# fdarmon/wild_deep_mvs

Measured on AMD Instinct MI355X. Metric: cost-volume voxels/sec (BxDxHxW), MVSNet hot path, higher is better.
Workload: dtype bf16

## Files before the change

### wild_deep_mvs_amd/csrc/conv3d_sweep.hip

```cpp
#include "conv_common.h"
#include <type_traits>

namespace pscv {

struct SweepArgs : ConvIO {
    int D, Hh, W;
    int epi;
    const uint16_t* in2;
    int in2_cs, in2_co;
    int nth, ntw, ndc, dc;
    unsigned mg_th, mg_tw, mg_dc;
};

PSCV_PROF_BUFFER(sweep)
constexpr int SW_BW = 18;
constexpr int SW_VB = 64;
constexpr int SW_NSLOT = 6;
template <int TH> struct SwGeom {
    static constexpr int BH = TH + 2;
    static constexpr int PV = ((BH * SW_BW + 7) / 8) * 8;
    static constexpr int PB = PV * SW_VB;
    static constexpr int LDS = SW_NSLOT * PB;
    static constexpr int CHUNKS = BH * SW_BW * 4;
    static constexpr int THREADS = 32 * TH;
    static constexpr int NLD = (CHUNKS + THREADS - 1) / THREADS;
};

__device__ __forceinline__ int sw_lds_off(int v, int chunk) {
    return v * SW_VB + ((chunk ^ (((v >> 2) & 1) << 1)) << 4);
}

template <typename H, int SW_TH>
__global__ __launch_bounds__(32 * SW_TH, 2) void conv3d_sweep8_kernel(const SweepArgs a) {
    extern __shared__ __attribute__((aligned(16))) unsigned char smem[];
    using G = SwGeom<SW_TH>;
    constexpr int SW_PB = G::PB, SW_CHUNKS = G::CHUNKS, NTHR = G::THREADS, NLD = G::NLD;
    constexpr int R = 2;

    int wg = xcd_remap(blockIdx.x, gridDim.x);
    const int dci = fast_divmod(wg, a.ndc, a.mg_dc);
    const int twi = fast_divmod(wg, a.ntw, a.mg_tw);
    const int thi = fast_divmod(wg, a.nth, a.mg_th);
    const int b = wg;
    const int h0 = thi * SW_TH, w0 = twi * 16;
    const int dbeg = dci * a.dc, dend = min(a.D, dbeg + a.dc);

    const int tid = threadIdx.x, lane = tid & 63, wave = tid >> 6;
    const int n = lane & 15, g = lane >> 4;
    PSCV_PROF_BEGIN

    uint4 wf[4][9];
    {
        const uint4* wp = reinterpret_cast<const uint4*>(a.wpk);
#pragma unroll
        for (int p = 0; p < 4; ++p)
#pragma unroll
            for (int t = 0; t < 9; ++t) wf[p][t] = wp[(p * 9 + t) * 64 + lane];
    }

    const int row0 = wave * R;
    int boff[R + 2][3];
#pragma unroll
    for (int rr = 0; rr < R + 2; ++rr)
#pragma unroll
        for (int kw = 0; kw < 3; ++kw) boff[rr][kw] = sw_lds_off((row0 + rr) * SW_BW + n + kw, g);

    unsigned goff[NLD];
    int loff[NLD];
    bool lval[NLD];
    const long plane_stride = (long)a.Hh * a.W * a.in_cs;
    const unsigned plane_bytes = (unsigned)(plane_stride * 2 - a.in_co * 2);
    const uint16_t* inb = a.in + (long)b * a.D * plane_stride + a.in_co;
#pragma unroll
    for (int i = 0; i < NLD; ++i) {
        const int id = tid + NTHR * i;
        const int v = id >> 2, c = id & 3;
        const int bh = v / SW_BW, bw = v - bh * SW_BW;
        const int gh = h0 - 1 + bh, gw = w0 - 1 + bw;
        lval[i] = id < SW_CHUNKS;
        const bool gval = lval[i] && (unsigned)gh < (unsigned)a.Hh && (unsigned)gw < (unsigned)a.W;
        goff[i] = gval ? ((unsigned)(gh * a.W + gw) * (unsigned)a.in_cs + (unsigned)(c * 8)) * 2u : 0x7ffffff0u;
        loff[i] = sw_lds_off(v, c);
    }
    const int plane_hi = min(a.D - 1, dend);
    auto fetch = [&](int plane, uint4 (&reg)[NLD]) {
        const bool pv = plane >= 0 && plane <= plane_hi;
        const __amdgpu_buffer_rsrc_t rs = __builtin_amdgcn_make_buffer_rsrc(
            const_cast<uint16_t*>(inb + (long)(pv ? plane : 0) * plane_stride), (short)0, pv ? (int)plane_bytes : 0, 0x00020000);
#pragma unroll
        for (int i = 0; i < NLD; ++i)
            reg[i] = __builtin_bit_cast(uint4, __builtin_amdgcn_raw_buffer_load_b128(rs, (int)goff[i], 0, 0));
    };
    auto stash = [&](int ring, const uint4 (&reg)[NLD]) {
        unsigned char* sp = smem + ring * SW_PB;
#pragma unroll
        for (int i = 0; i < NLD; ++i)
            if (lval[i]) *reinterpret_cast<uint4*>(sp + loff[i]) = reg[i];
    };

    const int c0 = (g & 1) * 4;
    float sc[4], bi[4], fl[4];
#pragma unroll
    for (int k = 0; k < 4; ++k) {
        sc[k] = a.scale ? a.scale[c0 + k] : 1.0f;
        bi[k] = a.bias ? a.bias[c0 + k] : 0.0f;
        fl[k] = a.floor ? a.floor[c0 + k] : 0.0f;
    }

    {
        uint4 ra[NLD], rb[NLD];
        fetch(dbeg - 1, ra); fetch(dbeg, rb);
        stash(0, ra); stash(1, rb);
        fetch(dbeg + 1, ra); fetch(dbeg + 2, rb);
        stash(2, ra); stash(3, rb);
    }
    __syncthreads();
    PSCV_STAMP(0)

    auto pair = [&](auto ringc, const int d) {
        constexpr int RING = decltype(ringc)::value;
        uint4 na[NLD], nb[NLD];
        fetch(d + 3, na);
        fetch(d + 4, nb);
        __builtin_amdgcn_sched_barrier(0);
        PSCV_STAMP(1)

        f32x4 acc[R];
#pragma unroll
        for (int r = 0; r < R; ++r) acc[r] = f32x4{0.f, 0.f, 0.f, 0.f};
#pragma unroll
        for (int p = 0; p < 4; ++p) {
            constexpr int SL = (RING + 4 * SW_NSLOT) % SW_NSLOT;
            const unsigned char* sp = smem + ((SL + p) % SW_NSLOT) * SW_PB;
#pragma unroll
            for (int kh = 0; kh < 3; ++kh)
#pragma unroll
                for (int kw = 0; kw < 3; ++kw)
#pragma unroll
                    for (int r = 0; r < R; ++r) {
                        const uint4 xf = *reinterpret_cast<const uint4*>(sp + boff[r + kh][kw]);
                        acc[r] = Mfma<H>::run(wf[p][kh * 3 + kw], xf, acc[r]);
                    }
        }

        PSCV_STAMP(2)
        const int od = d + (g >> 1);
#pragma unroll
        for (int r = 0; r < R; ++r) {
            const int oh = h0 + row0 + r, ow = w0 + n;
            if (od < dend && oh < a.Hh && ow < a.W) {
                const long vox = (((long)b * a.D + od) * a.Hh + oh) * a.W + ow;
                float y[4];
#pragma unroll
                for (int k = 0; k < 4; ++k) {
                    y[k] = fmaf(acc[r][k], sc[k], bi[k]);
                    if (a.epi & PSCV_EPI_RELU_PRE) y[k] = relu_floor(y[k], fl[k]);
                }
                if (a.skip) {
                    const uint2 sv = *reinterpret_cast<const uint2*>(a.skip + vox * a.skip_cs + a.skip_co + c0);
                    y[0] += Half16<H>::lo(sv.x); y[1] += Half16<H>::hi(sv.x);
                    y[2] += Half16<H>::lo(sv.y); y[3] += Half16<H>::hi(sv.y);
                }
                if (a.epi & PSCV_EPI_RELU_POST) {
#pragma unroll
                    for (int k = 0; k < 4; ++k) y[k] = relu_floor(y[k], 0.0f);
                }
                if (a.out_f32) {
                    *reinterpret_cast<float4*>(reinterpret_cast<float*>(a.out) + vox * a.out_cs + a.out_co + c0) =
                        make_float4(y[0], y[1], y[2], y[3]);
                } else {
                    *reinterpret_cast<uint2*>(reinterpret_cast<uint16_t*>(a.out) + vox * a.out_cs + a.out_co + c0) =
                        make_uint2(Half16<H>::pack(y[0], y[1]), Half16<H>::pack(y[2], y[3]));
                }
            }
        }

        PSCV_STAMP(3)
        stash((RING + 4) % SW_NSLOT, na);
        stash((RING + 5) % SW_NSLOT, nb);
        PSCV_STAMP(4)
        __syncthreads();
        PSCV_STAMP(5)
    };
    for (int d = dbeg; d < dend; d += 6) {
        pair(std::integral_constant<int, 0>{}, d);
        if (d + 2 < dend) pair(std::integral_constant<int, 2>{}, d + 2);
        if (d + 4 < dend) pair(std::integral_constant<int, 4>{}, d + 4);
    }
    PSCV_PROF_END(sweep, blockIdx.x)
}


constexpr int KM_NSLOT = 3;
constexpr int KM_PV = 192;
constexpr int KM_PB = KM_PV * SW_VB;
constexpr int KM_LDS = KM_NSLOT * KM_PB + 96;
constexpr int KM_CHUNKS = 10 * SW_BW * 4;
constexpr int KM_NLD = (KM_CHUNKS + 255) / 256;

#ifdef PSCV_ABLATE
#define KM_ABL(bit) (a.in2_cs & (bit))
#else
#define KM_ABL(bit) false
#endif
__device__ __forceinline__ int km_lds_off(int v, int chunk) { return v * SW_VB + ((chunk ^ ((v >> 2) & 3)) << 4); }

template <typename H, bool SKIP, int PD>
__global__ __launch_bounds__(256, 3) void conv3d_sweep8_kdm_kernel(const SweepArgs a) {
    extern __shared__ __attribute__((aligned(16))) unsigned char smem[];
    constexpr int NLD = KM_NLD;

    int wg = xcd_remap(blockIdx.x, gridDim.x);
    const int dci = fast_divmod(wg, a.ndc, a.mg_dc);
    const int twi = fast_divmod(wg, a.ntw, a.mg_tw);
    const int thi = fast_divmod(wg, a.nth, a.mg_th);
    const int b = wg;
    const int h0 = thi * 8, w0 = twi * 16;
    const int dbeg = dci * a.dc, dend = min(a.D, dbeg + a.dc);

    const int tid = threadIdx.x, lane = tid & 63, wave = tid >> 6;
    const int half = lane >> 5, nn = lane & 31;
    const int quad = nn >> 2;
    const int rr = ((0x69 >> quad) & 1) ? 0 : 1;
    const int px = (quad >> 1) * 4 + (nn & 3);
    const int row0 = wave * 2;

    uint4 wf[9][2];
    {
        const uint4* wp = reinterpret_cast<const uint4*>(a.wpk);
        const int kdb = nn >> 3, co = nn & 7;
#pragma unroll
        for (int t = 0; t < 9; ++t)
#pragma unroll
            for (int h = 0; h < 2; ++h)
                wf[t][h] = kdb < 3 ? wp[(kdb * 9 + t) * 64 + (2 * h + half) * 16 + co] : make_uint4(0u, 0u, 0u, 0u);
    }

    int boff[3][3];
#pragma unroll
    for (int kh = 0; kh < 3; ++kh)
#pragma unroll
        for (int kw = 0; kw < 3; ++kw) boff[kh][kw] = km_lds_off((row0 + rr + kh) * SW_BW + px + kw, half);

    unsigned goff[NLD];
    static_assert(NLD == 3 && KM_CHUNKS > 512 && KM_CHUNKS <= 768, "three chunks per thread, the third one partial");
    const int loff0 = km_lds_off(tid >> 2, tid & 3);
    const bool lval_last = tid + 512 < KM_CHUNKS;
    const long plane_stride = (long)a.Hh * a.W * a.in_cs;
    const unsigned plane_bytes = (unsigned)(plane_stride * 2 - a.in_co * 2);
    const uint16_t* inb = a.in + (long)b * a.D * plane_stride + a.in_co;
#pragma unroll
    for (int i = 0; i < NLD; ++i) {
        const int id = tid + 256 * i;
        const int v = id >> 2, c = id & 3;
        const int bh = v / SW_BW, bw = v - bh * SW_BW;
        const int gh = h0 - 1 + bh, gw = w0 - 1 + bw;
        const bool gval = id < KM_CHUNKS && (unsigned)gh < (unsigned)a.Hh && (unsigned)gw < (unsigned)a.W;
        goff[i] = gval ? ((unsigned)(gh * a.W + gw) * (unsigned)a.in_cs + (unsigned)(c * 8)) * 2u : 0x7ffffff0u;
    }
    const int plane_hi = min(a.D - 1, dend);
    auto fetch = [&](int plane, uint4 (&reg)[NLD]) {
        const bool pv = plane >= 0 && plane <= plane_hi;
        const __amdgpu_buffer_rsrc_t rs = __builtin_amdgcn_make_buffer_rsrc(
            const_cast<uint16_t*>(inb + (long)(pv ? plane : 0) * plane_stride), (short)0, pv ? (int)plane_bytes : 0, 0x00020000);
#pragma unroll
        for (int i = 0; i < NLD; ++i)
            reg[i] = __builtin_bit_cast(uint4, __builtin_amdgcn_raw_buffer_load_b128(rs, (int)goff[i], 0, 0));
    };
    auto stash = [&](int ring, const uint4 (&reg)[NLD]) {
        unsigned char* sp = smem + ring * KM_PB + loff0;
        *reinterpret_cast<uint4*>(sp) = reg[0];
        *reinterpret_cast<uint4*>(sp + 4096) = reg[1];
        if (lval_last) *reinterpret_cast<uint4*>(sp + 8192) = reg[2];
    };

    const int c0 = half * 4;
    float* const epc = reinterpret_cast<float*>(smem + KM_NSLOT * KM_PB);
    if (tid < 24) {
        const int k = tid & 7, which = tid >> 3;
        epc[tid] = which == 0 ? (a.scale ? a.scale[k] : 1.0f) : which == 1 ? (a.bias ? a.bias[k] : 0.0f) : (a.floor ? a.floor[k] : 0.0f);
    }
    const int oh = h0 + row0 + rr, ow = w0 + px;
    const bool pix_ok = oh < a.Hh && ow < a.W;
    const long vrow = ((long)b * a.D * a.Hh + oh) * a.W + ow;
    const long vplane = (long)a.Hh * a.W;
    auto fetch_skip = [&](int od) -> uint2 {
        uint2 sv = make_uint2(0u, 0u);
        if (SKIP && pix_ok && od >= dbeg && od < dend)
            sv = *reinterpret_cast<const uint2*>(a.skip + (vrow + od * vplane) * a.skip_cs + a.skip_co + c0);
        return sv;
    };
    auto epilogue = [&](int od, float d0, float d1, float d2, float d3, const uint2 sv) {
        if (!pix_ok) return;
        const long vox = vrow + od * vplane;
        float y[4] = {d0, d1, d2, d3};
        const float4 sc4 = *reinterpret_cast<const float4*>(epc + c0), bi4 = *reinterpret_cast<const float4*>(epc + 8 + c0);
        const float4 fl4 = *reinterpret_cast<const float4*>(epc + 16 + c0);
        const float sc[4] = {sc4.x, sc4.y, sc4.z, sc4.w}, bi[4] = {bi4.x, bi4.y, bi4.z, bi4.w}, fl[4] = {fl4.x, fl4.y, fl4.z, fl4.w};
#pragma unroll
        for (int k = 0; k < 4; ++k) {
            y[k] = fmaf(y[k], sc[k], bi[k]);
            if (a.epi & PSCV_EPI_RELU_PRE) y[k] = relu_floor(y[k], fl[k]);
        }
        if (SKIP) {
            y[0] += Half16<H>::lo(sv.x); y[1] += Half16<H>::hi(sv.x);
            y[2] += Half16<H>::lo(sv.y); y[3] += Half16<H>::hi(sv.y);
        }
        if (a.epi & PSCV_EPI_RELU_POST) {
#pragma unroll
            for (int k = 0; k < 4; ++k) y[k] = relu_floor(y[k], 0.0f);
        }
        if (a.out_f32) {
            *reinterpret_cast<float4*>(reinterpret_cast<float*>(a.out) + vox * a.out_cs + a.out_co + c0) = make_float4(y[0], y[1], y[2], y[3]);
        } else {
            *reinterpret_cast<uint2*>(reinterpret_cast<uint16_t*>(a.out) + vox * a.out_cs + a.out_co + c0) =
                make_uint2(Half16<H>::pack(y[0], y[1]), Half16<H>::pack(y[2], y[3]));
        }
    };

    uint4 nx[PD][NLD];
    {
        uint4 ra[NLD];
        fetch(dbeg - 1, ra);
#pragma unroll
        for (int s = 0; s < PD; ++s) fetch(dbeg + s, nx[s]);
        stash(0, ra);
    }
    __syncthreads();

    f32x16 acc;
#pragma unroll
    for (int k = 0; k < 16; ++k) acc[k] = 0.0f;
    uint2 skv = make_uint2(0u, 0u);
    int sl = 0;
    for (int p0 = dbeg - 1; p0 <= dend; p0 += PD) {
#pragma unroll
        for (int s = 0; s < PD; ++s) {
            const int p = p0 + s;
            if (p > dend) break;
            int sn = sl + 1;
            sn = sn >= KM_NSLOT ? 0 : sn;
            stash(sn, nx[s]);
            const uint2 skc = skv;
            skv = fetch_skip(p - 1);
            if (!KM_ABL(1) || p < dbeg) fetch(p + 1 + PD, nx[s]);
            __builtin_amdgcn_sched_barrier(0);

            const float d0 = acc[8], d1 = acc[9], d2 = acc[10], d3 = acc[11];
            acc[8] = acc[4]; acc[9] = acc[5]; acc[10] = acc[6]; acc[11] = acc[7];
            acc[4] = acc[0]; acc[5] = acc[1]; acc[6] = acc[2]; acc[7] = acc[3];
            acc[0] = 0.0f; acc[1] = 0.0f; acc[2] = 0.0f; acc[3] = 0.0f;

            const unsigned char* sp = smem + sl * KM_PB;
            if (!KM_ABL(4)) {
                constexpr int AH = 3;
                uint4 xb[AH];
#pragma unroll
                for (int t = 0; t < AH; ++t) xb[t] = *reinterpret_cast<const uint4*>(sp + (boff[(t >> 1) / 3][(t >> 1) % 3] ^ ((t & 1) << 5)));
#pragma unroll
                for (int t = 0; t < 18; ++t) {
                    acc = Mfma32<H>::run(wf[t >> 1][t & 1], xb[t % AH], acc);
                    if (t + AH < 18) {
                        const int u = t + AH;
                        xb[t % AH] = *reinterpret_cast<const uint4*>(sp + (boff[(u >> 1) / 3][(u >> 1) % 3] ^ ((u & 1) << 5)));
                    }
                }
                __builtin_amdgcn_sched_group_barrier(0x100, AH, 0);
#pragma unroll
                for (int t = 0; t < 18; ++t) {
                    __builtin_amdgcn_sched_group_barrier(0x008, 1, 0);
                    if (t + AH < 18) __builtin_amdgcn_sched_group_barrier(0x100, 1, 0);
                }
            }

            if (p - 2 >= dbeg && (!KM_ABL(2) || d0 == 123.456f)) epilogue(p - 2, d0, d1, d2, d3, skc);
            sl = sn;
            __syncthreads();
        }
    }
    epilogue(dend - 1, acc[8], acc[9], acc[10], acc[11], skv);
}

template <int CIN> struct ScGeom {
    static constexpr int VB = CIN * 2, CCH = CIN / 8;
    static constexpr int BH = 10, PV = 192;
    static constexpr int PB = PV * VB;
    static constexpr int LDS = SW_NSLOT * PB;
    static constexpr int CHUNKS = BH * SW_BW * CCH;
    static constexpr int NLD = (CHUNKS + 255) / 256;
    static constexpr int NM = 4 * 9 * CIN / 32;
};

template <typename H, int CIN, int PD, int COUT = 8>
__global__ __launch_bounds__(256, (CIN == 8 && PD <= 2) ? 4 : (CIN == 8 || (PD == 1 && COUT == 8)) ? 3 : 2) void conv3d_sweepc_kernel(const SweepArgs a) {
    static_assert(COUT == 8 || (COUT == 16 && CIN == 16), "narrow sweep: 8|16 -> 8 or 16 -> 16");
    constexpr int NOP = COUT == 16 ? 2 : 1;
    extern __shared__ __attribute__((aligned(16))) unsigned char smem[];
    using G = ScGeom<CIN>;
    constexpr int VB = G::VB, CCH = G::CCH, PB = G::PB, CHUNKS = G::CHUNKS, NLD = G::NLD, NM = G::NM;
    constexpr int R = 2;

    int wg = xcd_remap(blockIdx.x, gridDim.x);
    const int dci = fast_divmod(wg, a.ndc, a.mg_dc);
    const int twi = fast_divmod(wg, a.ntw, a.mg_tw);
    const int thi = fast_divmod(wg, a.nth, a.mg_th);
    const int b = wg;
    const int h0 = thi * 8, w0 = twi * 16;
    const int dbeg = dci * a.dc, dend = min(a.D, dbeg + a.dc);

    const int tid = threadIdx.x, lane = tid & 63, wave = tid >> 6;
    const int n = lane & 15, g = lane >> 4;

    uint4 wf[NM];
    {
        const uint4* wp = reinterpret_cast<const uint4*>(a.wpk);
#pragma unroll
        for (int m = 0; m < NM; ++m) wf[m] = wp[m * 64 + lane];
    }

    const int row0 = wave * R;
    int boff[R + 2][3];
#pragma unroll
    for (int rr = 0; rr < R + 2; ++rr)
#pragma unroll
        for (int kw = 0; kw < 3; ++kw) boff[rr][kw] = ((row0 + rr) * SW_BW + n + kw) * VB + (CIN == 16 ? (g & 1) * 16 : 0);
    const int pl0 = CIN == 8 ? g : (g >> 1);

    static_assert(NLD == CCH, "one load per 16-byte chunk of a voxel");
    unsigned goff[NLD];
    int loff[NLD];
    bool lval[NLD];
    long plane_stride[NLD];
    unsigned plane_bytes[NLD];
    const uint16_t* inb[NLD];
    {
        const int v = tid;
        const int bh = v / SW_BW, bw = v - bh * SW_BW;
        const int gh = h0 - 1 + bh, gw = w0 - 1 + bw;
        const bool in_tile = v < G::BH * SW_BW;
        const bool gval = in_tile && (unsigned)gh < (unsigned)a.Hh && (unsigned)gw < (unsigned)a.W;
#pragma unroll
        for (int i = 0; i < NLD; ++i) {
            const int cs = i == 0 ? a.in_cs : a.in2_cs, co = i == 0 ? a.in_co : a.in2_co;
            const uint16_t* base = i == 0 ? a.in : a.in2;
            lval[i] = in_tile;
            plane_stride[i] = (long)a.Hh * a.W * cs;
            plane_bytes[i] = (unsigned)(plane_stride[i] * 2 - co * 2);
            inb[i] = base + (long)b * a.D * plane_stride[i] + co;
            goff[i] = gval ? (unsigned)(gh * a.W + gw) * (unsigned)cs * 2u : 0x7ffffff0u;
            loff[i] = v * VB + i * 16;
        }
    }
    const int plane_hi = min(a.D - 1, dend);
    auto fetch = [&](int plane, uint4 (&reg)[NLD]) {
        const bool pv = plane >= 0 && plane <= plane_hi;
#pragma unroll
        for (int i = 0; i < NLD; ++i) {
            const __amdgpu_buffer_rsrc_t rs = __builtin_amdgcn_make_buffer_rsrc(
                const_cast<uint16_t*>(inb[i] + (long)(pv ? plane : 0) * plane_stride[i]), (short)0, pv ? (int)plane_bytes[i] : 0, 0x00020000);
            reg[i] = __builtin_bit_cast(uint4, __builtin_amdgcn_raw_buffer_load_b128(rs, (int)goff[i], 0, 0));
        }
    };
    auto stash = [&](int ring, const uint4 (&reg)[NLD]) {
        unsigned char* sp = smem + ring * PB;
#pragma unroll
        for (int i = 0; i < NLD; ++i)
            if (lval[i]) *reinterpret_cast<uint4*>(sp + loff[i]) = reg[i];
    };

    const int c0 = COUT == 16 ? g * 4 : (g & 1) * 4;
    float sc[4], bi[4], fl[4];
#pragma unroll
    for (int k = 0; k < 4; ++k) {
        sc[k] = a.scale ? a.scale[c0 + k] : 1.0f;
        bi[k] = a.bias ? a.bias[c0 + k] : 0.0f;
        fl[k] = a.floor ? a.floor[c0 + k] : 0.0f;
    }
    const bool col_ok = w0 + n < a.W;
    long vrow[R];
    bool row_ok[R];
#pragma unroll
    for (int r = 0; r < R; ++r) {
        row_ok[r] = col_ok && h0 + row0 + r < a.Hh;
        vrow[r] = ((long)b * a.D * a.Hh + (h0 + row0 + r)) * a.W + w0 + n;
    }
    const long vplane = (long)a.Hh * a.W;
    auto fetch_skip = [&](int dd, uint2 (&reg)[NOP][R]) {
#pragma unroll
        for (int op = 0; op < NOP; ++op) {
            const int od = COUT == 16 ? dd + op : dd + (g >> 1);
#pragma unroll
            for (int r = 0; r < R; ++r) {
                reg[op][r] = make_uint2(0u, 0u);
                if (a.skip && od < dend && row_ok[r])
                    reg[op][r] = *reinterpret_cast<const uint2*>(a.skip + (vrow[r] + od * vplane) * a.skip_cs + a.skip_co + c0);
            }
        }
    };

    {
        uint4 ra[NLD], rb[NLD];
        fetch(dbeg - 1, ra); fetch(dbeg, rb);
        stash(0, ra); stash(1, rb);
        fetch(dbeg + 1, ra); fetch(dbeg + 2, rb);
        stash(2, ra); stash(3, rb);
    }
    uint4 pfa[PD][NLD], pfb[PD][NLD];
    uint2 sk[PD][NOP][R];
#pragma unroll
    for (int s = 0; s < PD; ++s) {
        fetch(dbeg + 3 + 2 * s, pfa[s]);
        fetch(dbeg + 4 + 2 * s, pfb[s]);
        fetch_skip(dbeg + 2 * s, sk[s]);
    }
    __syncthreads();

    int ring = 0;
    for (int d = dbeg; d < dend; d += 2 * PD) {
#pragma unroll
        for (int s = 0; s < PD; ++s) {
            const int dd = d + 2 * s;
            if (dd < dend) {
                int s4 = ring + 4, s5 = ring + 5;
                s4 = s4 >= SW_NSLOT ? s4 - SW_NSLOT : s4;
                s5 = s5 >= SW_NSLOT ? s5 - SW_NSLOT : s5;
                stash(s4, pfa[s]);
                stash(s5, pfb[s]);
                fetch(dd + 3 + 2 * PD, pfa[s]);
                fetch(dd + 4 + 2 * PD, pfb[s]);

                f32x4 acc[NOP][R];
#pragma unroll
                for (int op = 0; op < NOP; ++op)
#pragma unroll
                    for (int r = 0; r < R; ++r) acc[op][r] = f32x4{0.f, 0.f, 0.f, 0.f};
#pragma unroll
                for (int op = 0; op < NOP; ++op)
#pragma unroll
                    for (int set = 0; set < NM / 9; ++set) {
                        int sl = ring + pl0 + (COUT == 16 ? op + set : 2 * set);
                        sl = sl >= SW_NSLOT ? sl - SW_NSLOT : sl;
                        const unsigned char* sp = smem + sl * PB;
#pragma unroll
                        for (int kh = 0; kh < 3; ++kh) {
#pragma unroll
                            for (int kw = 0; kw < 3; ++kw)
#pragma unroll
                                for (int r = 0; r < R; ++r) {
                                    const uint4 xf = *reinterpret_cast<const uint4*>(sp + boff[r + kh][kw]);
                                    acc[op][r] = Mfma<H>::run(wf[set * 9 + kh * 3 + kw], xf, acc[op][r]);
                                }
                            if (COUT == 16) __builtin_amdgcn_sched_barrier(0);
                        }
                    }

#pragma unroll
                for (int op = 0; op < NOP; ++op) {
                    const int od = COUT == 16 ? dd + op : dd + (g >> 1);
#pragma unroll
                    for (int r = 0; r < R; ++r) {
                        if (od < dend && row_ok[r]) {
                            const long vox = vrow[r] + od * vplane;
                            float y[4];
#pragma unroll
                            for (int k = 0; k < 4; ++k) {
                                y[k] = fmaf(acc[op][r][k], sc[k], bi[k]);
                                if (a.epi & PSCV_EPI_RELU_PRE) y[k] = relu_floor(y[k], fl[k]);
                            }
                            if (a.skip) {
                                y[0] += Half16<H>::lo(sk[s][op][r].x); y[1] += Half16<H>::hi(sk[s][op][r].x);
                                y[2] += Half16<H>::lo(sk[s][op][r].y); y[3] += Half16<H>::hi(sk[s][op][r].y);
                            }
                            if (a.epi & PSCV_EPI_RELU_POST) {
#pragma unroll
                                for (int k = 0; k < 4; ++k) y[k] = relu_floor(y[k], 0.0f);
                            }
                            if (a.out_f32) {
                                *reinterpret_cast<float4*>(reinterpret_cast<float*>(a.out) + vox * a.out_cs + a.out_co + c0) =
                                    make_float4(y[0], y[1], y[2], y[3]);
                            } else {
                                *reinterpret_cast<uint2*>(reinterpret_cast<uint16_t*>(a.out) + vox * a.out_cs + a.out_co + c0) =
                                    make_uint2(Half16<H>::pack(y[0], y[1]), Half16<H>::pack(y[2], y[3]));
                            }
                        }
                    }
                }
                fetch_skip(dd + 2 * PD, sk[s]);
                ring += 2;
                ring = ring >= SW_NSLOT ? ring - SW_NSLOT : ring;
                __syncthreads();
            }
        }
    }
}

template <typename H, int CIN, int PD, int COUT = 8>
static int sweepc_launch_t(SweepArgs& a, long nblk, hipStream_t st) {
    return launch("pscv_conv3d(sweep)", conv3d_sweepc_kernel<H, CIN, PD, COUT>, dim3((unsigned)nblk), dim3(256), ScGeom<CIN>::LDS, st, a);
}
template <typename H, int CIN, int COUT = 8>
static int sweepc_launch_pd(SweepArgs& a, long nblk, hipStream_t st) {
    const int pd = g_sweepc_pd > 0 ? g_sweepc_pd : (COUT == 16 ? 2 : 1);
    return pd == 1 ? sweepc_launch_t<H, CIN, 1, COUT>(a, nblk, st) : pd == 2 ? sweepc_launch_t<H, CIN, 2, COUT>(a, nblk, st)
                                                                             : sweepc_launch_t<H, CIN, 3, COUT>(a, nblk, st);
}

static void sweep_args(SweepArgs& a, const ConvCall& c, int th) {
    static_cast<ConvIO&>(a) = c.io;
    a.D = c.D; a.Hh = c.H; a.W = c.W; a.epi = c.epi;
    a.nth = (c.H + th - 1) / th;
    a.ntw = (c.W + 15) / 16;
}

int conv3d_sweepc_launch(const ConvCall& c) {
    PSCV_CHECK_ARG((long)c.H * c.W * c.io.in_cs * 2 < 0x7fffffffL, "pscv_conv3d(sweep): an input plane of %d x %d x %d channels exceeds 2 GiB", c.H, c.W, c.io.in_cs);
    PSCV_CHECK_ARG(!c.in2 || (c.c_in == 16 && (long)c.H * c.W * c.in2_cs * 2 < 0x7fffffffL), "pscv_conv3d(sweep): a second input tensor needs c_in = 16 and planes below 2 GiB");
    SweepArgs a;
    sweep_args(a, c, 8);
    a.in2 = c.in2 ? c.in2 : a.in;
    a.in2_cs = c.in2 ? c.in2_cs : a.in_cs;
    a.in2_co = c.in2 ? c.in2_co : a.in_co + 8;
    const long slots = g_sweepc_slots > 0 ? g_sweepc_slots : (c.c_out == 16 ? 512 : 768);
    a.dc = plan_depth_chunk(c.D, (long)a.B * a.nth * a.ntw, slots, 4, true, g_sweep_dc);
    a.ndc = (c.D + a.dc - 1) / a.dc;
    const long nblk = finish_grid("pscv_conv3d(sweep)", a.B, a.nth, a.ntw, a.ndc, a.mg_th, a.mg_tw, a.mg_dc);
    if (nblk < 0) return -1;
    return with_half("pscv_conv3d(sweep)", c.dtype, [&](auto t) {
        using H = typename decltype(t)::type;
        if (c.c_out == 16) return sweepc_launch_pd<H, 16, 16>(a, nblk, c.st);
        return c.c_in == 8 ? sweepc_launch_pd<H, 8>(a, nblk, c.st) : sweepc_launch_pd<H, 16>(a, nblk, c.st);
    });
}

int conv3d_sweep8_launch(const ConvCall& c) {
    PSCV_CHECK_ARG((long)c.H * c.W * c.io.in_cs * 2 < 0x7fffffffL, "pscv_conv3d(sweep): an input plane of %d x %d x %d channels exceeds 2 GiB", c.H, c.W, c.io.in_cs);
    const bool kdm = g_sweep_kdm != 0;
    const bool tall = !kdm && g_sweep_th16 && c.H >= 16;
    SweepArgs a;
    sweep_args(a, c, tall ? 16 : 8);
    const long tiles = (long)a.B * a.nth * a.ntw;
    if (kdm) {
#ifdef PSCV_ABLATE
        a.in2_cs = g_fuse_c0;
#endif
        a.dc = plan_depth_chunk(c.D, tiles, g_sweep_kdm >= 2 ? 1024 : 768, 4, false, g_sweep_dc);
    } else {
        a.dc = plan_depth_chunk(c.D, tiles, tall ? 256 : 512, 4, true, g_sweep_dc);
    }
    a.ndc = (c.D + a.dc - 1) / a.dc;
    const long nblk = finish_grid("pscv_conv3d(sweep)", a.B, a.nth, a.ntw, a.ndc, a.mg_th, a.mg_tw, a.mg_dc);
    if (nblk < 0) return -1;
    const bool skip = c.io.skip != nullptr;
    const int pd = g_sweep_kdm_pd > 0 ? g_sweep_kdm_pd : 1;
    return with_half("pscv_conv3d(sweep)", c.dtype, [&](auto t) {
        using H = typename decltype(t)::type;
        const char* what = "pscv_conv3d(sweep)";
        const dim3 grid((unsigned)nblk);
        if (kdm && pd >= 2) return skip ? launch(what, conv3d_sweep8_kdm_kernel<H, true, 2>, grid, dim3(256), KM_LDS, c.st, a)
                                        : launch(what, conv3d_sweep8_kdm_kernel<H, false, 2>, grid, dim3(256), KM_LDS, c.st, a);
        if (kdm) return skip ? launch(what, conv3d_sweep8_kdm_kernel<H, true, 1>, grid, dim3(256), KM_LDS, c.st, a)
                             : launch(what, conv3d_sweep8_kdm_kernel<H, false, 1>, grid, dim3(256), KM_LDS, c.st, a);
        return tall ? launch(what, conv3d_sweep8_kernel<H, 16>, grid, dim3(512), SwGeom<16>::LDS, c.st, a)
                    : launch(what, conv3d_sweep8_kernel<H, 8>, grid, dim3(256), SwGeom<8>::LDS, c.st, a);
    });
}

}

PSCV_PROF_EXPORT(sweep)
```

Measured before the change: 13.29 billion.

## Use buffer stores with lane-swap packing and a specialised hot epilogue in sweep kernel

Rewrites the sweep8 kernel's output epilogue to use raw buffer loads and stores with precomputed 32-bit offsets. Out-of-range lanes get an offset beyond the buffer so the hardware drops them, which replaces the per-element bounds branches. For bf16 outputs it uses permlane16_swap to merge two rows' 8-byte results into one 16-byte store per lane. A compile-time HOT specialisation, for the no-skip relu-pre case, removes the runtime epilogue flags. Two new host checks require two output planes to fit in 2 GiB, and the swap path needs aligned output.

New measurement: 13.52 billion (median of 6 runs). +1.7%, better.

```diff
diff --git a/wild_deep_mvs_amd/csrc/conv3d_sweep.hip b/wild_deep_mvs_amd/csrc/conv3d_sweep.hip
--- a/wild_deep_mvs_amd/csrc/conv3d_sweep.hip
+++ b/wild_deep_mvs_amd/csrc/conv3d_sweep.hip
@@ -10,12 +10,15 @@
     int in2_cs, in2_co;
     int nth, ntw, ndc, dc;
     unsigned mg_th, mg_tw, mg_dc;
+    int st16;
 };
 
 PSCV_PROF_BUFFER(sweep)
 constexpr int SW_BW = 18;
 constexpr int SW_VB = 64;
 constexpr int SW_NSLOT = 6;
+typedef unsigned sw_u32x4 __attribute__((ext_vector_type(4)));
+typedef unsigned sw_u32x2 __attribute__((ext_vector_type(2)));
 template <int TH> struct SwGeom {
     static constexpr int BH = TH + 2;
     static constexpr int PV = ((BH * SW_BW + 7) / 8) * 8;
@@ -30,7 +33,7 @@
     return v * SW_VB + ((chunk ^ (((v >> 2) & 1) << 1)) << 4);
 }
 
-template <typename H, int SW_TH>
+template <typename H, int SW_TH, bool HOT>
 __global__ __launch_bounds__(32 * SW_TH, 2) void conv3d_sweep8_kernel(const SweepArgs a) {
     extern __shared__ __attribute__((aligned(16))) unsigned char smem[];
     using G = SwGeom<SW_TH>;
@@ -106,6 +109,32 @@
         bi[k] = a.bias ? a.bias[c0 + k] : 0.0f;
         fl[k] = a.floor ? a.floor[c0 + k] : 0.0f;
     }
+    const bool out_f32 = !HOT && a.out_f32, has_skip = !HOT && a.skip != nullptr, st16 = HOT || a.st16;
+    const bool relu_pre = HOT || (a.epi & PSCV_EPI_RELU_PRE), relu_post = !HOT && (a.epi & PSCV_EPI_RELU_POST);
+
+    constexpr unsigned OOR = 0x7ffffff0u;
+    const unsigned oes = out_f32 ? 4u : 2u;
+    const long oplane_b = (long)a.Hh * a.W * a.out_cs * oes, splane_b = (long)a.Hh * a.W * a.skip_cs * 2;
+    const char* outb = reinterpret_cast<const char*>(a.out) + (long)b * a.D * oplane_b + a.out_co * oes;
+    const char* skb = reinterpret_cast<const char*>(a.skip) + (long)b * a.D * splane_b + a.skip_co * 2;
+    unsigned ooff[R], soff[R], ooff16;
+    {
+        const int ow = w0 + n;
+#pragma unroll
+        for (int r = 0; r < R; ++r) {
+            const int oh = h0 + row0 + r;
+            const bool ok = oh < a.Hh && ow < a.W;
+            const unsigned pix = (unsigned)(oh * a.W + ow);
+            ooff[r] = ok ? (unsigned)(g >> 1) * (unsigned)oplane_b + (pix * (unsigned)a.out_cs + (unsigned)c0) * oes : OOR;
+            soff[r] = ok && has_skip ? (unsigned)(g >> 1) * (unsigned)splane_b + (pix * (unsigned)a.skip_cs + (unsigned)c0) * 2u : OOR;
+        }
+        const int oh = h0 + row0 + (g & 1);
+        ooff16 = oh < a.Hh && ow < a.W ? (unsigned)(g >> 1) * (unsigned)oplane_b + (unsigned)(oh * a.W + ow) * (unsigned)a.out_cs * 2u : OOR;
+    }
+    auto pair_rsrc = [&](const char* base, long plane_b, int co_b, int d) {
+        const int np = min(2, dend - d);
+        return __builtin_amdgcn_make_buffer_rsrc(const_cast<char*>(base + d * plane_b), (short)0, (int)(np * plane_b - co_b), 0x00020000);
+    };
 
     {
         uint4 ra[NLD], rb[NLD];
@@ -144,34 +173,43 @@
         }
 
         PSCV_STAMP(2)
-        const int od = d + (g >> 1);
+        const __amdgpu_buffer_rsrc_t ors = pair_rsrc(outb, oplane_b, (int)(a.out_co * oes), d);
+        uint2 sv[R];
+        if (has_skip) {
+            const __amdgpu_buffer_rsrc_t srs = pair_rsrc(skb, splane_b, a.skip_co * 2, d);
+#pragma unroll
+            for (int r = 0; r < R; ++r) sv[r] = __builtin_bit_cast(uint2, __builtin_amdgcn_raw_buffer_load_b64(srs, (int)soff[r], 0, 0));
+        }
+        uint2 pk[R];
 #pragma unroll
         for (int r = 0; r < R; ++r) {
-            const int oh = h0 + row0 + r, ow = w0 + n;
-            if (od < dend && oh < a.Hh && ow < a.W) {
-                const long vox = (((long)b * a.D + od) * a.Hh + oh) * a.W + ow;
-                float y[4];
-#pragma unroll
-                for (int k = 0; k < 4; ++k) {
-                    y[k] = fmaf(acc[r][k], sc[k], bi[k]);
-                    if (a.epi & PSCV_EPI_RELU_PRE) y[k] = relu_floor(y[k], fl[k]);
-                }
-                if (a.skip) {
-                    const uint2 sv = *reinterpret_cast<const uint2*>(a.skip + vox * a.skip_cs + a.skip_co + c0);
-                    y[0] += Half16<H>::lo(sv.x); y[1] += Half16<H>::hi(sv.x);
-                    y[2] += Half16<H>::lo(sv.y); y[3] += Half16<H>::hi(sv.y);
-                }
-                if (a.epi & PSCV_EPI_RELU_POST) {
-#pragma unroll
-                    for (int k = 0; k < 4; ++k) y[k] = relu_floor(y[k], 0.0f);
-                }
-                if (a.out_f32) {
-                    *reinterpret_cast<float4*>(reinterpret_cast<float*>(a.out) + vox * a.out_cs + a.out_co + c0) =
-                        make_float4(y[0], y[1], y[2], y[3]);
-                } else {
-                    *reinterpret_cast<uint2*>(reinterpret_cast<uint16_t*>(a.out) + vox * a.out_cs + a.out_co + c0) =
-                        make_uint2(Half16<H>::pack(y[0], y[1]), Half16<H>::pack(y[2], y[3]));
-                }
+            float y[4];
+#pragma unroll
+            for (int k = 0; k < 4; ++k) {
+                y[k] = fmaf(acc[r][k], sc[k], bi[k]);
+                if (relu_pre) y[k] = relu_floor(y[k], fl[k]);
+            }
+            if (has_skip) {
+                y[0] += Half16<H>::lo(sv[r].x); y[1] += Half16<H>::hi(sv[r].x);
+                y[2] += Half16<H>::lo(sv[r].y); y[3] += Half16<H>::hi(sv[r].y);
+            }
+            if (relu_post) {
+#pragma unroll
+                for (int k = 0; k < 4; ++k) y[k] = relu_floor(y[k], 0.0f);
+            }
+            if (out_f32)
+                __builtin_amdgcn_raw_buffer_store_b128(__builtin_bit_cast(sw_u32x4, make_float4(y[0], y[1], y[2], y[3])), ors, (int)ooff[r], 0, 0);
+            else
+                pk[r] = make_uint2(Half16<H>::pack(y[0], y[1]), Half16<H>::pack(y[2], y[3]));
+        }
+        if (!out_f32) {
+            if (st16) {
+                const auto rx = __builtin_amdgcn_permlane16_swap(pk[0].x, pk[1].x, false, false);
+                const auto ry = __builtin_amdgcn_permlane16_swap(pk[0].y, pk[1].y, false, false);
+                __builtin_amdgcn_raw_buffer_store_b128(sw_u32x4{rx[0], ry[0], rx[1], ry[1]}, ors, (int)ooff16, 0, 0);
+            } else {
+#pragma unroll
+                for (int r = 0; r < R; ++r) __builtin_amdgcn_raw_buffer_store_b64(sw_u32x2{pk[r].x, pk[r].y}, ors, (int)ooff[r], 0, 0);
             }
         }
 
@@ -610,6 +648,7 @@
     a.D = c.D; a.Hh = c.H; a.W = c.W; a.epi = c.epi;
     a.nth = (c.H + th - 1) / th;
     a.ntw = (c.W + 15) / 16;
+    a.st16 = 0;
 }
 
 int conv3d_sweepc_launch(const ConvCall& c) {
@@ -639,6 +678,13 @@
     SweepArgs a;
     sweep_args(a, c, tall ? 16 : 8);
     const long tiles = (long)a.B * a.nth * a.ntw;
+    if (!kdm) {
+        PSCV_CHECK_ARG(2L * c.H * c.W * c.io.out_cs * (c.io.out_f32 ? 4 : 2) < 0x7ffffff0L,
+                       "pscv_conv3d(sweep): two output planes of %d x %d x %d channels exceed 2 GiB", c.H, c.W, c.io.out_cs);
+        PSCV_CHECK_ARG(!c.io.skip || 2L * c.H * c.W * c.io.skip_cs * 2 < 0x7ffffff0L,
+                       "pscv_conv3d(sweep): two residual planes of %d x %d x %d channels exceed 2 GiB", c.H, c.W, c.io.skip_cs);
+        a.st16 = !c.io.out_f32 && c.io.out_cs % 8 == 0 && c.io.out_co % 8 == 0 && (reinterpret_cast<uintptr_t>(c.io.out) & 15) == 0;
+    }
     if (kdm) {
 #ifdef PSCV_ABLATE
         a.in2_cs = g_fuse_c0;
@@ -660,8 +706,10 @@
                                         : launch(what, conv3d_sweep8_kdm_kernel<H, false, 2>, grid, dim3(256), KM_LDS, c.st, a);
         if (kdm) return skip ? launch(what, conv3d_sweep8_kdm_kernel<H, true, 1>, grid, dim3(256), KM_LDS, c.st, a)
                              : launch(what, conv3d_sweep8_kdm_kernel<H, false, 1>, grid, dim3(256), KM_LDS, c.st, a);
-        return tall ? launch(what, conv3d_sweep8_kernel<H, 16>, grid, dim3(512), SwGeom<16>::LDS, c.st, a)
-                    : launch(what, conv3d_sweep8_kernel<H, 8>, grid, dim3(256), SwGeom<8>::LDS, c.st, a);
+        if (tall) return launch(what, conv3d_sweep8_kernel<H, 16, false>, grid, dim3(512), SwGeom<16>::LDS, c.st, a);
+        const bool hot = a.st16 && !skip && (c.epi & (PSCV_EPI_RELU_PRE | PSCV_EPI_RELU_POST)) == PSCV_EPI_RELU_PRE;
+        return hot ? launch(what, conv3d_sweep8_kernel<H, 8, true>, grid, dim3(256), SwGeom<8>::LDS, c.st, a)
+                   : launch(what, conv3d_sweep8_kernel<H, 8, false>, grid, dim3(256), SwGeom<8>::LDS, c.st, a);
     });
 }
 
```
